# braun-steven/DAFNe

Hardware: AMD Instinct MI355X
Metric: images/sec on 1024x1024 DOTA tiles, R101-FPN (higher is better)
Workload: dtype bf16; 1 GPU; DOTA-1.0 1024x1024 R101-FPN bf16, batch 8 per GPU (per-GPU shard of configs[2]; the model BASELINE.json's metric names), uint8 tiles resident in HBM -> detections; per_gpu_batch=8, global_batch=8, classes=15, parallelism=dp1 (independent images, RCCL gather of detections), mode=pipelined

## Files before the change

### dafne_amd/_lib.py

```python
import ctypes
import os

_HERE = os.path.dirname(os.path.abspath(__file__))
LIB_PATH = os.environ.get("DAFNE_AMD_LIB") or os.path.join(_HERE, "libdafne_amd.so")
_lib = None

c_void_p = ctypes.c_void_p
c_int = ctypes.c_int
c_i64 = ctypes.c_int64
c_size_t = ctypes.c_size_t
c_double = ctypes.c_double
c_float = ctypes.c_float
c_u32 = ctypes.c_uint32
c_i32 = ctypes.c_int32


class LevelDesc(ctypes.Structure):
    _fields_ = [("d_logits", c_void_p), ("d_delta", c_void_p), ("d_center", c_void_p),
                ("d_ctrness", c_void_p), ("logits_ps", c_i32), ("delta_ps", c_i32),
                ("center_ps", c_i32), ("ctrness_ps", c_i32), ("H", c_i32), ("W", c_i32), ("stride", c_i32),
                ("scale", c_float)]


class DecodeParams(ctypes.Structure):
# ... 73 lines not shown
    "dafne_abi_version": (c_int, []),
    "dafne_last_error": (ctypes.c_char_p, []),
    "dafne_poly_iou_pairs_hip": (c_int, [c_void_p, c_void_p, c_i64, c_void_p, c_void_p]),
    "dafne_poly_nms_workspace_bytes": (c_size_t, [c_int, c_int]),
    "dafne_poly_nms_stats_offset": (c_size_t, [c_int, c_int, c_int]),
    "dafne_poly_nms_hip": (c_int, [c_void_p, c_int, c_double, c_void_p, c_void_p, c_void_p, c_size_t, c_int, c_void_p]),
    "dafne_poly_nms_batched_hip": (c_int, [c_void_p, c_void_p, c_int, c_int, c_double, c_int, c_void_p,
                                           c_void_p, c_void_p, c_size_t, c_int, c_void_p]),
    "dafne_poly_nms_f64_workspace_bytes": (c_size_t, [c_int, c_int]),
    "dafne_poly_nms_f64_batched_hip": (c_int, [c_void_p, c_void_p, c_int, c_int, c_double, c_int, c_void_p,
                                               c_void_p, c_void_p, c_size_t, c_int, c_void_p]),
    "dafne_hbb_nms_f64_workspace_bytes": (c_size_t, [c_int, c_int]),
    "dafne_hbb_nms_f64_batched_hip": (c_int, [c_void_p, c_void_p, c_int, c_int, c_double, c_void_p, c_void_p, c_void_p, c_size_t,
                                              c_void_p]),
    "dafne_select_over_all_levels_hip": (c_int, [c_void_p, c_void_p, c_void_p, c_void_p, c_int, c_int,
                                                 c_double, c_int, c_void_p, c_void_p, c_void_p, c_size_t,
                                                 c_int, c_void_p]),
    "dafne_decode_workspace_bytes": (c_size_t, [ctypes.POINTER(DecodeParams), ctypes.POINTER(LevelDesc)]),
    "dafne_decode_levels_hip": (c_int, [ctypes.POINTER(DecodeParams), ctypes.POINTER(LevelDesc)] +
                                [c_void_p] * 8 + [c_void_p, c_size_t, c_void_p]),
    "dafne_sort_quadrilateral_hip": (c_int, [c_void_p, c_void_p, c_i64, c_void_p]),
    "dafne_corner_chain_hip": (c_int, [ctypes.POINTER(ChainSeg), c_int, c_int, c_int, c_void_p, c_void_p]),
    "dafne_gather_detections_hip": (c_int, [c_void_p] * 10 + [c_int, c_int, c_int, c_int, c_void_p, c_void_p,
                                                             c_void_p]),
    "dafne_conv2d_nhwc_bf16_hip": (c_int, [ctypes.POINTER(ConvParams), ctypes.POINTER(ConvSeg), c_void_p]),
    "dafne_conv2d_nhwc_fp8w_hip": (c_int, [ctypes.POINTER(ConvParams), ctypes.POINTER(ConvSeg), c_void_p, c_float, c_void_p]),
    "dafne_conv2d_num_tiles": (c_int, [ctypes.POINTER(ConvParams), ctypes.POINTER(ConvSeg)]),
    "dafne_conv2d_fp8w_num_tiles": (c_int, [ctypes.POINTER(ConvParams), ctypes.POINTER(ConvSeg)]),
    "dafne_conv2d_fp8w_tiles_per_image": (c_int, [ctypes.POINTER(ConvParams), ctypes.POINTER(ConvSeg), c_void_p]),
    "dafne_resize_workspace_bytes": (c_size_t, [c_int, c_int, c_int]),
    "dafne_resize_bilinear_u8_hip": (c_int, [c_void_p, c_int, c_int, c_int, c_int, c_int, c_int, c_int, c_int, c_void_p,
                                             c_void_p, c_size_t, c_void_p]),
    "dafne_conv2d_kernel_id": (c_int, [ctypes.POINTER(ConvParams), ctypes.POINTER(ConvSeg)]),
    "dafne_conv2d_tiles_per_image": (c_int, [ctypes.POINTER(ConvParams), ctypes.POINTER(ConvSeg), c_void_p]),
    "dafne_groupnorm_finalize_hip": (c_int, [ctypes.POINTER(GnSeg), c_int, c_int, c_int, c_void_p, c_void_p,
                                             ctypes.c_float, c_void_p]),
    "dafne_conv2d_cout_pad": (c_int, [c_int]),
    "dafne_conv2d_tile_pixels": (c_int, [ctypes.POINTER(ConvParams), ctypes.POINTER(ConvSeg)]),
    "dafne_preprocess_image_hip": (c_int, [c_void_p, c_int, c_int, c_int, c_int, c_void_p,
                                           ctypes.POINTER(c_float), ctypes.POINTER(c_float), c_int, c_int,
                                           c_void_p, c_void_p]),
    "dafne_conv3x3_c64_hip": (c_int, [c_void_p, c_void_p, c_void_p, c_int, c_int, c_int, c_int, c_void_p, c_void_p]),
    "dafne_conv3x3_c256_ok": (c_int, [ctypes.POINTER(ConvParams), ctypes.POINTER(ConvSeg)]),
    "dafne_conv3x3_c256_num_tiles": (c_int, [ctypes.POINTER(ConvParams), ctypes.POINTER(ConvSeg)]),
    "dafne_conv3x3_c256_tiles_per_image": (c_int, [ctypes.POINTER(ConvParams), ctypes.POINTER(ConvSeg), c_void_p]),
    "dafne_conv3x3_c256_pair_hip": (c_int, [ctypes.POINTER(ConvParams), ctypes.POINTER(ConvSeg), c_void_p,
                                            ctypes.POINTER(ConvParams), ctypes.POINTER(ConvSeg), c_void_p, c_void_p, c_size_t, c_void_p]),
    "dafne_conv3x3_c256_scratch_bytes": (c_size_t, []),
    "dafne_conv3x3_c256_hip": (c_int, [ctypes.POINTER(ConvParams), ctypes.POINTER(ConvSeg), c_void_p, c_void_p, c_size_t, c_void_p]),
    "dafne_conv2d_wr_ok": (c_int, [ctypes.POINTER(ConvParams), ctypes.POINTER(ConvSeg)]),
    "dafne_conv2d_wr_splits": (c_int, [ctypes.POINTER(ConvParams), ctypes.POINTER(ConvSeg)]),
    "dafne_conv2d_wr_workspace_bytes": (c_size_t, [ctypes.POINTER(ConvParams), ctypes.POINTER(ConvSeg)]),
    "dafne_conv2d_wr_hip": (c_int, [ctypes.POINTER(ConvParams), ctypes.POINTER(ConvSeg), c_void_p, c_void_p, c_size_t, c_void_p]),
    "dafne_bottleneck_body_scratch_bytes": (c_size_t, []),
    "dafne_bottleneck_body_hip": (c_int, [c_void_p, c_void_p, c_void_p, c_void_p, c_void_p, c_void_p, c_int, c_int, c_int,
                                          c_void_p, c_void_p, c_void_p, c_size_t, c_void_p]),
    "dafne_bottleneck_body16_hip": (c_int, [c_void_p, c_void_p, c_void_p, c_void_p, c_void_p, c_void_p, c_int, c_int, c_int,
                                            c_void_p, c_void_p, c_void_p, c_size_t, c_void_p]),
    "dafne_bottleneck_tail_head_hip": (c_int, [c_void_p, c_void_p, c_void_p, c_void_p, c_void_p, c_int, c_int, c_int,
                                               c_void_p, c_void_p, c_void_p]),
    "dafne_bottleneck_tail_head_narrow_hip": (c_int, [c_void_p, c_void_p, c_void_p, c_void_p, c_void_p, c_int, c_int, c_int,
                                                      c_void_p, c_void_p, c_void_p]),
    "dafne_bottleneck_tail_head_mid_hip": (c_int, [c_void_p, c_void_p, c_void_p, c_void_p, c_void_p, c_int, c_int, c_int,
                                                   c_void_p, c_void_p, c_void_p]),
    "dafne_bottleneck_proj_tail_head_narrow_hip": (c_int, [c_void_p, c_void_p, c_void_p, c_void_p, c_void_p, c_void_p, c_int,
                                                           c_int, c_int, c_void_p, c_void_p, c_void_p]),
    "dafne_bottleneck_block_narrow_scratch_bytes": (c_size_t, []),
    "dafne_bottleneck_block_narrow_hip": (c_int, [c_void_p] * 7 + [c_int, c_int, c_int, c_void_p, c_void_p, c_void_p, c_size_t, c_void_p]),
    "dafne_bottleneck_block_narrow_s2_scratch_bytes": (c_size_t, []),
    "dafne_bottleneck_block_narrow_s2_hip": (c_int, [c_void_p] * 5 + [c_int, c_int, c_int, c_void_p, c_void_p, c_size_t, c_void_p]),
    "dafne_bottleneck_block_mid_scratch_bytes": (c_size_t, []),
    "dafne_bottleneck_block_mid_hip": (c_int, [c_void_p] * 6 + [c_int, c_int, c_int, c_void_p, c_void_p, c_void_p, c_size_t, c_void_p]),
    "dafne_stem_pool_hip": (c_int, [c_void_p, c_void_p, c_void_p, c_int, c_int, c_int, c_void_p, c_void_p]),
    "dafne_stem_pool_conv1_hip": (c_int, [c_void_p, c_void_p, c_void_p, c_void_p, c_void_p, c_int, c_int, c_int, c_void_p, c_void_p,
                                          c_void_p]),
    "dafne_maxpool3x3s2_nhwc_bf16_hip": (c_int, [c_void_p, c_void_p, c_int, c_int, c_int, c_int, c_void_p]),
    "dafne_groupnorm_relu_nhwc_bf16_hip": (c_int, [ctypes.POINTER(GnSeg), c_int, c_int, c_int, c_void_p, c_void_p,
                                                   c_void_p, c_void_p, c_float, c_void_p]),
    "dafne_relu_copy_bf16_hip": (c_int, [c_void_p, c_void_p, c_i64, c_void_p]),
    "dafne_scene_tiles_workspace_bytes": (c_size_t, [c_int]),
    "dafne_scene_tiles_u8_hip": (c_int, [ctypes.POINTER(SceneTile), c_int, c_int, c_void_p, c_void_p, c_size_t, c_void_p]),
    "dafne_scene_merge_workspace_bytes": (c_size_t, [c_int, c_int]),
    "dafne_scene_merge_rows_hip": (c_int, [c_void_p, c_void_p, c_int, c_int, c_void_p, c_int, c_int, ctypes.c_uint64, c_int,
                                           c_int, c_void_p, c_void_p, c_void_p, c_void_p, c_size_t, c_void_p]),
    "dafne_scene_merge_hbb_rows_hip": (c_int, [c_void_p, c_void_p, c_int, c_int, c_void_p, c_int, c_int, ctypes.c_uint64, c_int,
                                               c_int, c_void_p, c_void_p, c_void_p, c_void_p, c_size_t, c_void_p]),
    "dafne_scene_views_workspace_bytes": (c_size_t, [ctypes.POINTER(ViewSrc), c_int, c_int, c_int]),
    "dafne_scene_views_u8_hip": (c_int, [ctypes.POINTER(ViewSrc), c_int, c_int, c_int, c_void_p, c_void_p, c_size_t, c_void_p]),
    "dafne_scene_scaled_tiles_workspace_bytes": (c_size_t, [ctypes.POINTER(ScaledTile), c_int]),
    "dafne_scene_scaled_tiles_u8_hip": (c_int, [ctypes.POINTER(ScaledTile), c_int, c_int, c_void_p, c_void_p, c_size_t, c_void_p]),
    "dafne_scene_merge_rows_scaled_hip": (c_int, [c_void_p, c_void_p, c_int, c_int, c_void_p, c_void_p, c_int, c_int,
                                                  ctypes.c_uint64, c_int, c_int, c_void_p, c_void_p, c_void_p, c_void_p, c_size_t,
                                                  c_void_p]),
    "dafne_scene_merge_hbb_rows_scaled_hip": (c_int, [c_void_p, c_void_p, c_int, c_int, c_void_p, c_void_p, c_int, c_int,
                                                      ctypes.c_uint64, c_int, c_int, c_void_p, c_void_p, c_void_p, c_void_p,
                                                      c_size_t, c_void_p]),
    "dafne_tta_candidates_workspace_bytes": (c_size_t, [c_int, c_int]),
    "dafne_tta_candidates_hip": (c_int, [ctypes.POINTER(TtaView), c_int, c_int, c_int, c_int] + [c_void_p] * 10 + [c_size_t, c_void_p]),
    "dafne_scene_match_hip": (c_int, [c_void_p, c_void_p, c_int, c_void_p, c_void_p, c_int, c_int, c_void_p, c_void_p, c_void_p]),
    "dafne_scene_match_hbb_hip": (c_int, [c_void_p, c_void_p, c_int, c_void_p, c_void_p, c_int, c_int, c_void_p, c_void_p, c_void_p]),
    "dafne_scene_mark_workspace_bytes": (c_size_t, [c_int]),
    "dafne_scene_mark_hip": (c_int, [c_void_p, c_void_p, c_void_p, c_void_p, c_int, c_void_p, c_int, c_void_p, c_int, c_double,
                                     c_void_p, c_void_p, c_void_p, c_size_t, c_void_p]),
    "dafne_assign_targets_hip": (c_int, [ctypes.POINTER(TargetParams)] + [c_void_p] * 5 + [c_int] + [c_void_p] * 6),
    "dafne_losses_workspace_bytes": (c_size_t, [ctypes.POINTER(LossParams), ctypes.POINTER(LevelDesc)]),
    "dafne_losses_hip": (c_int, [ctypes.POINTER(LossParams), ctypes.POINTER(LevelDesc)] + [c_void_p] * 7 + [c_size_t, c_void_p]),
# ... 46 lines not shown
```

### dafne_amd/csrc/abi.hip

```cpp
#include "common.h"

namespace dafne {
char* err_buf() {
    static thread_local char buf[512] = {0};
    return buf;
}
}

extern "C" {
int dafne_abi_version(void) { return 151; }
const char* dafne_last_error(void) { return dafne::err_buf(); }
}
```

### dafne_amd/engine.py

```python
import ctypes

import torch

from . import _lib
from .engine_options import EngineOptions

BF16 = torch.bfloat16
STAGE_BLOCKS = {50: (3, 4, 6, 3), 101: (3, 4, 23, 3)}

F_RELU, F_RES, F_UP, F_F32, F_GN, F_GNIN, F_GNFIN, F_EXCL = 1, 2, 4, 8, 16, 32, 64, 128
F_FRAG16 = 256
F_RELU_INPUT = 512
FPN_IN_FEATURES = ("res3", "res4", "res5")


class Act:

    __slots__ = ("t", "n", "h", "w", "c")

    def __init__(self, n, h, w, c, device):
        self.t = torch.zeros(n, h + 2, w + 2, c, dtype=BF16, device=device)
        self.n, self.h, self.w, self.c = n, h, w, c

    def nchw_float(self):
# ... 174 lines not shown
    return 8 * a + 4 * cb + i


def pack_bneck16(w2, w3, w1):
    assert tuple(w2.shape) == (256, 2304) and w2.dtype == BF16
    assert tuple(w3.shape) == (1024, 256) and tuple(w1.shape) == (256, 1024) and w3.dtype == BF16 and w1.dtype == BF16
    perm = _bneck_row_perm16(w2.device)
    a0 = w2.reshape(8, 32, 72, 4, 8)[:, perm].reshape(8, 2, 16, 72, 4, 8).permute(0, 3, 1, 4, 2, 5)
    a1 = w3.reshape(4, 8, 32, 8, 4, 8)[:, :, perm].reshape(4, 8, 2, 16, 8, 4, 8).permute(0, 1, 4, 2, 5, 3, 6)
    a2 = w1.reshape(8, 32, 4, 8, 4, 8)[:, perm].reshape(8, 2, 16, 4, 8, 4, 8).permute(3, 0, 4, 1, 5, 2, 6)
    pb = torch.stack([a1, a2], dim=1).contiguous().reshape(-1)
    return torch.cat([a0.contiguous().reshape(-1), pb]).contiguous()


def bneck_weights(P, key, w2, w3, w1):
    f16 = P["options"].rp_mfma16
    fkey, other = (key + "bneck16", key + "bneck") if f16 else (key + "bneck", key + "bneck16")
    assert other not in P, "one conv_bneck form per model: %s" % other
    if fkey not in P:
        P[fkey] = pack_bneck16(w2, w3, w1) if f16 else pack_bneck(w2, w3, w1)
    return P[fkey], f16


def pack_conv3x3_frag(w):
    cout = w.shape[0]
    assert w.dim() == 2 and w.shape[1] == 2304 and cout % 256 == 0 and w.dtype == BF16
    return w.reshape(cout // 256, 8, 32, 144, 2, 8).permute(0, 1, 3, 4, 2, 5).contiguous().reshape(-1)


def pack_conv3x3_frag16(w):
    cout = w.shape[0]
    assert w.dim() == 2 and w.shape[1] == 2304 and cout % 256 == 0 and w.dtype == BF16
    return w.reshape(cout // 256, 8, 2, 16, 72, 4, 8).permute(0, 1, 4, 2, 5, 3, 6).contiguous().reshape(-1)


def pack_rp(w, options=None):
    options = options or EngineOptions.from_env()
    return (pack_conv3x3_frag16(w), F_FRAG16) if options.rp_mfma16 else (pack_conv3x3_frag(w), 0)


def rp_weights(P, key, wgt):
    f16 = P["options"].rp_mfma16
    fkey, other = (key + ".frag16", key + ".frag") if f16 else (key + ".frag", key + ".frag16")
    assert other not in P, "one resident-patch form per model: %s" % other
    if fkey not in P:
        P[fkey] = pack_rp(wgt, P["options"])[0]
    return P[fkey], f16


def pack_conv_frag(w):
    cout, k = w.shape
    assert w.dim() == 2 and cout % 256 == 0 and k % 64 == 0 and w.dtype == BF16
    return w.reshape(cout // 256, 8, 32, k // 16, 2, 8).permute(0, 1, 3, 4, 2, 5).contiguous().reshape(-1)


FP8_KERNELS = ("patch",)


_RP_SCRATCH = {}


def rp_scratch(device):
    key = str(device)
    if key not in _RP_SCRATCH:
        _RP_SCRATCH[key] = torch.empty(_lib.load().dafne_conv3x3_c256_scratch_bytes(), dtype=torch.uint8, device=device)
    return _RP_SCRATCH[key]


def pack_b2b_narrow(w3, w1, wsc=None):
    assert tuple(w3.shape) == (256, 64) and tuple(w1.shape) == (64, 256) and w3.dtype == BF16 and w1.dtype == BF16
    parts = [w3.reshape(8, 32, 4, 2, 8).permute(0, 2, 3, 1, 4).reshape(-1),
             w1.reshape(2, 32, 16, 2, 8).permute(0, 2, 3, 1, 4).reshape(-1)]
    if wsc is not None:
        assert tuple(wsc.shape) == (256, 64) and wsc.dtype == BF16
        parts.append(wsc.reshape(8, 32, 4, 2, 8).permute(0, 2, 3, 1, 4).reshape(-1))
    return torch.cat(parts).contiguous()


def pack_blk_narrow(w2, w3, w1=None, wsc=None):
    assert tuple(w2.shape) == (64, 576) and tuple(w3.shape) == (256, 64) and w2.dtype == BF16 and w3.dtype == BF16
    a2 = w2.reshape(2, 32, 36, 2, 8).permute(0, 2, 3, 1, 4).reshape(-1)

    def quarters(w):
        return w.reshape(2, 4, 32, 4, 2, 8).permute(0, 1, 3, 4, 2, 5).reshape(-1)
    if w1 is not None:
        assert tuple(w1.shape) == (64, 256) and w1.dtype == BF16
        a1 = w1.reshape(2, 32, 16, 2, 8).permute(0, 2, 3, 1, 4).reshape(-1)
    else:
        a1 = torch.zeros(2 * 16 * 64 * 8, dtype=BF16, device=w2.device)
    if wsc is not None:
        assert tuple(wsc.shape) == (256, 64) and wsc.dtype == BF16
        asc = quarters(wsc)
    else:
        asc = torch.zeros(256 * 64, dtype=BF16, device=w2.device)
    return torch.cat([a2, quarters(w3), a1, asc]).contiguous()


def pack_blk_mid(w2, w3, w1=None):
    assert tuple(w2.shape) == (128, 1152) and tuple(w3.shape) == (512, 128) and w2.dtype == BF16 and w3.dtype == BF16
    a2 = w2.reshape(4, 32, 72, 2, 8).permute(0, 2, 3, 1, 4).reshape(-1)
    a3 = w3.reshape(2, 8, 32, 8, 2, 8).permute(0, 1, 3, 4, 2, 5).reshape(-1)
    if w1 is not None:
        assert tuple(w1.shape) == (128, 512) and w1.dtype == BF16
        a1 = w1.reshape(4, 32, 32, 2, 8).permute(0, 2, 3, 1, 4).reshape(-1)
    else:
        a1 = torch.zeros(128 * 512, dtype=BF16, device=w2.device)
# ... 118 lines not shown
        rc = _lib.load().dafne_conv3x3_c256_pair_hip(ctypes.byref(a.prm), a.segs, _lib.ptr(a.wfrag), ctypes.byref(b.prm), b.segs,
                                                     _lib.ptr(b.wfrag), _lib.ptr(scr), scr.numel(), stream)
        if rc:
            _lib.check(rc, "dafne_conv3x3_c256_pair_hip")


WR_NOMINAL_BATCH = 8


def wr_takes(k, stride, cin, cout, npx):
    if k == 3:
        return stride in (1, 2) and npx <= 10000 and cin in (256, 512) and cout == cin
    if stride == 1:
        return (cin == 512 and cout == 2048 and npx <= 10000) or (cout == 256 and cin >= 1024 and npx <= 40000)
    return cin == 512 and cout == 256 and npx <= 40000


class WrWorkspace:

    def __init__(self, device):
        self.device, self.bytes, self.t = device, 0, None

    def need(self, nbytes):
        assert self.t is None
        self.bytes = max(self.bytes, int(nbytes))

    def tensor(self):
        if self.t is None:
            self.t = torch.zeros(max(self.bytes, 1 << 16), dtype=torch.uint8, device=self.device)
        return self.t


class WrCall:

    def __init__(self, conv, wfrag, ws):
        self.conv, self.wfrag, self.ws = conv, wfrag, ws
        self.prm, self.segs = conv.prm, conv.segs
        self.flops, self.bytes = conv.flops, conv.bytes
        L = _lib.load()
        self.splits = L.dafne_conv2d_wr_splits(ctypes.byref(self.prm), self.segs)
        assert self.splits >= 1
        ws.need(L.dafne_conv2d_wr_workspace_bytes(ctypes.byref(self.prm), self.segs))

    def kernel_name(self):
        return "conv_wr"

    def __call__(self, stream):
        w = self.ws.tensor()
        rc = _lib.load().dafne_conv2d_wr_hip(ctypes.byref(self.prm), self.segs, _lib.ptr(self.wfrag), _lib.ptr(w), w.numel(), stream)
        if rc:
            _lib.check(rc, "dafne_conv2d_wr_hip")


class FnCall:
    def __init__(self, fn, args, keep, name, flops=0, nbytes=0):
        self.fn, self.args, self.keep, self.name = fn, args, keep, name
        self.flops, self.bytes = flops, nbytes

    def kernel_name(self):
        return self.name

    def __call__(self, stream):
        rc = self.fn(*self.args, stream)
        if rc:
            _lib.check(rc, self.name)


def conv_out_hw(h, w, k, stride, pad):
    return (h + 2 * pad - k) // stride + 1, (w + 2 * pad - k) // stride + 1


class DensePlan:

    def __init__(self, weights, n, h, w, depth, num_classes, device, with_head=True, head_outputs=None, calib=None,
                 shared_gpu=False):
        assert h % 32 == 0 and w % 32 == 0
        self.shared_gpu = bool(shared_gpu)
        self._build(weights, n, h, w, depth, num_classes, device, with_head, head_outputs, calib)

    def _build(self, weights, n, h, w, depth, num_classes, device, with_head, head_outputs, calib):
        self.calib = calib
        self.n, self.h, self.w = n, h, w
        self.device = device
        self.calls = []
        self.flops = 0
        self.graph = None
        L = _lib.load()
        P = weights
        pool = Pool(device)
        self.pool = pool

        opt = P["options"]
        shared = self.shared_gpu and not opt.shared_excl
        act_q8 = P.get("act_q8") or {}
        wr_on = opt.conv_wr
        self.wr_ws = WrWorkspace(device)
        use_c64 = opt.conv_c64
        inplace_res = opt.inplace_res

        def res_dead(sc_, x_, b_):
            if not inplace_res or sc_ is None:
                return False
            if b_ == 0:
                return sc_ is not x_
            return not any(sc_ is f for f in feats.values())

        def conv(key, tin, k, stride, pad, flags, res=None, out=None, cout=None):
            wgt, bias = P[key]
            cin = tin.c
            cout = cout or wgt.shape[0]
            ho, wo = conv_out_hw(tin.h, tin.w, k, stride, pad)
            o = out or pool.get(n, ho, wo, cout)
            if (use_c64 and k == 3 and stride == 1 and pad == 1 and cin == 64 and cout == 64 and res is None
                    and (flags & ~F_RELU) == 0 and tuple(wgt.shape) == (64, 576) and bias is not None):
                fl = 2 * n * ho * wo * 64 * 576
                self.calls.append(FnCall(L.dafne_conv3x3_c64_hip,
                                         (_lib.ptr(tin.t), _lib.ptr(wgt), _lib.ptr(bias), n, ho, wo, 1 if flags & F_RELU else 0, _lib.ptr(o.t)),
                                         (tin, wgt, bias, o), "conv3x3_c64", flops=fl,
                                         nbytes=2 * n * ho * wo * 64 * 2 + wgt.numel() * 2))
                self.flops += fl
                return o
            q8 = P.get(key + ".fp8")
            fp8 = None
            if q8 is not None and k == 3 and stride == 1 and res is None and not (flags & (F_F32 | F_UP | F_RES)):
                if calib is not None:
                    self.calls.append(AmaxProbe(calib, key, [tin]))
                elif key in act_q8:
                    fp8 = (q8[1] / act_q8[key], act_q8[key])
            c = ConvCall(q8[0] if fp8 else wgt, bias, cin, cout, k, stride, pad, flags,
                         [(tin.t, o.t, res.t if res is not None else None, tin.h, tin.w, ho, wo)], n, fp8=fp8,
                         shared_gpu=shared)
            if (fp8 is None and wr_on and wr_takes(k, stride, cin, cout, WR_NOMINAL_BATCH * ho * wo) and bias is not None
                    and L.dafne_conv2d_wr_ok(ctypes.byref(c.prm), c.segs)):
                if key + ".wr" not in P:
                    P[key + ".wr"] = pack_conv_frag(wgt)
                w = WrCall(c, P[key + ".wr"], self.wr_ws)
                self.calls.append(w)
                self.flops += w.flops
                return o
            assert not (flags & F_RELU_INPUT), "only conv_wr rectifies its input on load (the caller checks wr_takes)"
            if fp8 is None and k == 3 and cin == 256 and opt.conv_rp and c.kernel_id() == 6 and c.rp_ok():
                wfrag, f16 = rp_weights(P, key, wgt)
                c = ConvCall(wgt, bias, cin, cout, k, stride, pad, flags,
                             [(tin.t, o.t, None, tin.h, tin.w, ho, wo)], n, wfrag=wfrag, shared_gpu=shared, frag16=f16)
            self.calls.append(c)
            self.flops += c.flops
            return o

        self.stem_in = torch.zeros(n, h + 6, w + 6, 4, dtype=BF16, device=device)
        wgt, bias = P["stem"]
        x = pool.get(n, h // 4, w // 4, 64)
        stem_flops = 2 * n * (h // 2) * (w // 2) * 64 * 7 * 7 * 3
        stem_y1 = None
        if opt.fuse_stem:
            c1 = P.get("res2.0.conv1")
            if (opt.fuse_stem_conv1 and c1 is not None and tuple(c1[0].shape) == (64, 64)
                    and c1[1] is not None):
                stem_y1 = pool.get(n, h // 4, w // 4, 64)
                c1_flops = 2 * n * (h // 4) * (w // 4) * 64 * 64
                fc = FnCall(L.dafne_stem_pool_conv1_hip, (_lib.ptr(self.stem_in), _lib.ptr(wgt), _lib.ptr(bias), _lib.ptr(c1[0]),
                                                          _lib.ptr(c1[1]), n, h, w, _lib.ptr(x.t), _lib.ptr(stem_y1.t)),
                            (self.stem_in, wgt, bias, c1[0], c1[1], x, stem_y1), "stem_pool_conv1", flops=stem_flops + c1_flops,
                            nbytes=n * ((h + 6) * (w + 6) * 8 + (h // 4) * (w // 4) * 256))
                self.calls.append(fc)
                self.flops += stem_flops + c1_flops
            else:
                fc = FnCall(L.dafne_stem_pool_hip, (_lib.ptr(self.stem_in), _lib.ptr(wgt), _lib.ptr(bias), n, h, w, _lib.ptr(x.t)),
                            (self.stem_in, wgt, bias, x), "stem_pool", flops=stem_flops,
                            nbytes=n * ((h + 6) * (w + 6) * 8 + (h // 4) * (w // 4) * 128))
                self.calls.append(fc)
                self.flops += stem_flops
        else:
            stem_out = pool.get(n, h // 2, w // 2, 64)
            c = ConvCall(wgt, bias, 4, 64, 7, 2, 3, F_RELU,
                         [(self.stem_in, stem_out.t, None, h + 6, w + 6, h // 2, w // 2)], n, shared_gpu=shared)
            self.calls.append(c)
            self.flops += c.flops
            self.calls.append(FnCall(L.dafne_maxpool3x3s2_nhwc_bf16_hip,
                                     (_lib.ptr(stem_out.t), _lib.ptr(x.t), n, h // 2, w // 2, 64),
                                     (stem_out, x), "maxpool"))
            pool.put(stem_out)

        feats = {}
        fuse_b2b, fuse_narrow, fuse_mid, fuse_bneck = opt.fuse_b2b, opt.b2b_narrow_on, opt.b2b_mid_on, opt.bneck_on
# ... 555 lines not shown
```

### include/dafne_amd.h

```cpp
#ifndef DAFNE_AMD_H
#define DAFNE_AMD_H

#include <stddef.h>
#include <stdint.h>

#ifdef __cplusplus
extern "C" {
#endif

#define DAFNE_OK 0
#define DAFNE_E_INVALID 1
#define DAFNE_E_WORKSPACE 2
#define DAFNE_E_HIP 3
#define DAFNE_E_UNSUPPORTED 4

int dafne_abi_version(void);
const char* dafne_last_error(void);

int dafne_poly_iou_pairs_hip(const double* d_p, const double* d_q, int64_t n,
                             double* d_out, void* stream);

size_t dafne_poly_nms_f64_workspace_bytes(int n_images, int m_cap);
int dafne_poly_nms_f64_batched_hip(const double* d_dets9, const int32_t* d_counts, int n_images, int m_cap,
                                   double thresh, int strict_hbb, int64_t* d_keep, int32_t* d_num_keep,
// ... 53 lines not shown
                                const int64_t* d_keep, const int32_t* d_num_keep,
                                const float* d_sizes, int do_postprocess, int n_images, int m_cap,
                                int k_cap, float* d_out, int32_t* d_out_counts, void* stream);

#define DAFNE_CONV_RELU 1u
#define DAFNE_CONV_RESIDUAL 2u
#define DAFNE_CONV_UPSAMPLE_ADD 4u
#define DAFNE_CONV_OUT_F32 8u
#define DAFNE_CONV_GN_STATS 16u
#define DAFNE_CONV_GN_INPUT 32u
#define DAFNE_CONV_GN_FINALIZE 64u
#define DAFNE_CONV_EXCLUSIVE 128u

#define DAFNE_CONV_FRAG16 256u
#define DAFNE_CONV_RELU_INPUT 512u

typedef struct dafne_conv_seg {
    const void* d_in;
    void* d_out;
    const void* d_res;
    int32_t Hin, Win, Hout, Wout;
} dafne_conv_seg;

typedef struct dafne_conv_params {
    int32_t n_images, n_segs;
    int32_t Cin, Cout, KH, KW, stride, pad;
    uint32_t flags;
    const void* d_weight;
    const float* d_bias;
    float* d_gn_partial;
    const float* d_in_gn_stats;
    const float* d_in_gn_gamma;
    const float* d_in_gn_beta;
    float* d_gn_stats_out;
    int32_t* d_gn_counters;
    float gn_eps;
} dafne_conv_params;

int dafne_conv2d_nhwc_bf16_hip(const dafne_conv_params* prm, const dafne_conv_seg* segs, void* stream);
int dafne_conv3x3_c256_ok(const dafne_conv_params* prm, const dafne_conv_seg* segs);
int dafne_conv3x3_c256_num_tiles(const dafne_conv_params* prm, const dafne_conv_seg* segs);
int dafne_conv3x3_c256_tiles_per_image(const dafne_conv_params* prm, const dafne_conv_seg* segs, int32_t* out);
int dafne_conv3x3_c256_pair_hip(const dafne_conv_params* prm_a, const dafne_conv_seg* segs_a, const void* d_wfrag_a,
                                const dafne_conv_params* prm_b, const dafne_conv_seg* segs_b, const void* d_wfrag_b,
                                void* d_scratch, size_t scratch_bytes, void* stream);
size_t dafne_conv3x3_c256_scratch_bytes(void);
int dafne_conv3x3_c256_hip(const dafne_conv_params* prm, const dafne_conv_seg* segs, const void* d_wfrag, void* d_scratch,
                           size_t scratch_bytes, void* stream);
int dafne_conv2d_wr_ok(const dafne_conv_params* prm, const dafne_conv_seg* segs);
int dafne_conv2d_wr_splits(const dafne_conv_params* prm, const dafne_conv_seg* segs);
size_t dafne_conv2d_wr_workspace_bytes(const dafne_conv_params* prm, const dafne_conv_seg* segs);
int dafne_conv2d_wr_hip(const dafne_conv_params* prm, const dafne_conv_seg* segs, const void* d_wfrag, void* d_workspace,
                        size_t workspace_bytes, void* stream);
int dafne_conv2d_nhwc_fp8w_hip(const dafne_conv_params* prm, const dafne_conv_seg* segs, const float* d_oscale,
                               float in_qscale, void* stream);
int dafne_conv2d_fp8w_num_tiles(const dafne_conv_params* prm, const dafne_conv_seg* segs);
int dafne_conv2d_fp8w_tiles_per_image(const dafne_conv_params* prm, const dafne_conv_seg* segs, int32_t* out);
int dafne_conv2d_cout_pad(int Cout);
int dafne_conv2d_tile_pixels(const dafne_conv_params* prm, const dafne_conv_seg* segs);
int dafne_conv2d_num_tiles(const dafne_conv_params* prm, const dafne_conv_seg* segs);
int dafne_conv2d_kernel_id(const dafne_conv_params* prm, const dafne_conv_seg* segs);
int dafne_conv2d_tiles_per_image(const dafne_conv_params* prm, const dafne_conv_seg* segs, int32_t* out);

int dafne_preprocess_image_hip(const uint8_t* d_img, int layout_hwc, int n_images, int H, int W,
                               const int32_t* d_valid_hw, const float* mean3, const float* std3,
                               int Hn, int Wn, void* d_out, void* stream);
size_t dafne_resize_workspace_bytes(int C, int H, int new_w);
int dafne_resize_bilinear_u8_hip(const uint8_t* d_in, int layout_hwc, int C, int H, int W, int new_h, int new_w,
                                 int hflip, int vflip, uint8_t* d_out, void* d_ws, size_t ws_bytes, void* stream);
int dafne_conv3x3_c64_hip(const void* d_in, const void* d_weight, const float* d_bias, int n_images, int H, int W, int relu,
                          void* d_out, void* stream);
int dafne_bottleneck_tail_head_hip(const void* d_in, const void* d_res, const void* d_wfrag, const float* d_bias3,
                                   const float* d_bias1, int n_images, int H, int W, void* d_out, void* d_next,
                                   void* stream);
size_t dafne_bottleneck_body_scratch_bytes(void);
int dafne_bottleneck_body_hip(const void* d_in, const void* d_res, const void* d_wfrag, const float* d_bias2,
                              const float* d_bias3, const float* d_bias1, int n_images, int H, int W, void* d_out,
                              void* d_next, void* d_scratch, size_t scratch_bytes, void* stream);
int dafne_bottleneck_body16_hip(const void* d_in, const void* d_res, const void* d_wfrag, const float* d_bias2,
                                const float* d_bias3, const float* d_bias1, int n_images, int H, int W, void* d_out,
                                void* d_next, void* d_scratch, size_t scratch_bytes, void* stream);
int dafne_bottleneck_tail_head_narrow_hip(const void* d_in, const void* d_res, const void* d_wfrag, const float* d_bias3,
                                          const float* d_bias1, int n_images, int H, int W, void* d_out, void* d_next,
                                          void* stream);
int dafne_bottleneck_tail_head_mid_hip(const void* d_in, const void* d_res, const void* d_wfrag, const float* d_bias3,
                                       const float* d_bias1, int n_images, int H, int W, void* d_out, void* d_next,
                                       void* stream);
int dafne_bottleneck_proj_tail_head_narrow_hip(const void* d_in, const void* d_x0, const void* d_wfrag, const float* d_bias3,
                                               const float* d_bias_sc, const float* d_bias1, int n_images, int H, int W,
                                               void* d_out, void* d_next, void* stream);
size_t dafne_bottleneck_block_narrow_scratch_bytes(void);
int dafne_bottleneck_block_narrow_hip(const void* d_in, const void* d_res, const void* d_wfrag, const float* d_bias2,
                                      const float* d_bias3, const float* d_bias_sc, const float* d_bias1, int n_images, int H, int W,
                                      void* d_out, void* d_next, void* d_scratch, size_t scratch_bytes, void* stream);
size_t dafne_bottleneck_block_narrow_s2_scratch_bytes(void);
int dafne_bottleneck_block_narrow_s2_hip(const void* d_in, const void* d_res, const void* d_wfrag, const float* d_bias2,
                                         const float* d_bias3, int n_images, int H, int W, void* d_out, void* d_scratch,
                                         size_t scratch_bytes, void* stream);
size_t dafne_bottleneck_block_mid_scratch_bytes(void);
int dafne_bottleneck_block_mid_hip(const void* d_in, const void* d_res, const void* d_wfrag, const float* d_bias2,
                                   const float* d_bias3, const float* d_bias1, int n_images, int H, int W, void* d_out,
                                   void* d_next, void* d_scratch, size_t scratch_bytes, void* stream);
int dafne_stem_pool_hip(const void* d_in, const void* d_weight, const float* d_bias, int n_images, int H, int W,
                        void* d_out, void* stream);
int dafne_stem_pool_conv1_hip(const void* d_in, const void* d_weight, const float* d_bias, const void* d_w1, const float* d_b1,
                              int n_images, int H, int W, void* d_out, void* d_out1, void* stream);
// ... 144 lines not shown
```

Baseline: 1420 images/sec.

## Add dedicated persistent MFMA GEMM kernel for 1x1 convs with 512->256 channels

Adds a new HIP kernel that runs 1x1 convolutions as a persistent GEMM. It keeps weights in registers, streams input pixels into LDS through a three-stage global_load_lds pipeline, uses XCD-aware tile walkers, and fuses bias, residual or top-down add, and ReLU into an LDS-staged epilogue. The engine routes only the stride-1 512->256 1x1 layer (the FPN res3 lateral) to this kernel, ahead of the existing conv_wr path. The aim is to cut the generic conv overhead for this layer, at the cost of a large amount of new inline-asm code that must hold correct wait counts and swizzles.

After: 1425 images/sec (median of 6 runs). No clear change (+0.4%).

```diff
diff --git a/dafne_amd/_lib.py b/dafne_amd/_lib.py
--- a/dafne_amd/_lib.py
+++ b/dafne_amd/_lib.py
@@ -149,6 +149,9 @@
     "dafne_conv2d_wr_splits": (c_int, [ctypes.POINTER(ConvParams), ctypes.POINTER(ConvSeg)]),
     "dafne_conv2d_wr_workspace_bytes": (c_size_t, [ctypes.POINTER(ConvParams), ctypes.POINTER(ConvSeg)]),
     "dafne_conv2d_wr_hip": (c_int, [ctypes.POINTER(ConvParams), ctypes.POINTER(ConvSeg), c_void_p, c_void_p, c_size_t, c_void_p]),
+    "dafne_conv1x1_gemm_ok": (c_int, [ctypes.POINTER(ConvParams), ctypes.POINTER(ConvSeg)]),
+    "dafne_conv1x1_gemm_tiles": (ctypes.c_longlong, [ctypes.POINTER(ConvParams), ctypes.POINTER(ConvSeg)]),
+    "dafne_conv1x1_gemm_hip": (c_int, [ctypes.POINTER(ConvParams), ctypes.POINTER(ConvSeg), c_void_p, c_void_p]),
     "dafne_bottleneck_body_scratch_bytes": (c_size_t, []),
     "dafne_bottleneck_body_hip": (c_int, [c_void_p, c_void_p, c_void_p, c_void_p, c_void_p, c_void_p, c_int, c_int, c_int,
                                           c_void_p, c_void_p, c_void_p, c_size_t, c_void_p]),
diff --git a/dafne_amd/csrc/abi.hip b/dafne_amd/csrc/abi.hip
--- a/dafne_amd/csrc/abi.hip
+++ b/dafne_amd/csrc/abi.hip
@@ -8,6 +8,6 @@
 }
 
 extern "C" {
-int dafne_abi_version(void) { return 151; }
+int dafne_abi_version(void) { return 152; }
 const char* dafne_last_error(void) { return dafne::err_buf(); }
 }
diff --git a/dafne_amd/csrc/conv1x1_gemm.hip b/dafne_amd/csrc/conv1x1_gemm.hip
--- /dev/null
+++ b/dafne_amd/csrc/conv1x1_gemm.hip
@@ -0,0 +1,444 @@
+#include <type_traits>
+
+#include "common.h"
+
+namespace {
+
+typedef __attribute__((ext_vector_type(8))) __bf16 bf16x8;
+typedef __attribute__((ext_vector_type(16))) float f32x16;
+typedef __attribute__((ext_vector_type(4))) float f32x4;
+typedef __attribute__((ext_vector_type(4))) unsigned u32x4;
+typedef __attribute__((ext_vector_type(2))) unsigned u32x2;
+typedef __attribute__((address_space(1))) void gvoid;
+typedef __attribute__((address_space(3))) void lvoid;
+
+template <int NW, int KR>
+struct Cfg {
+    static constexpr int NT = 64 * NW, CT = 32 * NW;
+    static constexpr int PX = KR ? 64 : 128;
+    static constexpr int PF = PX / 32;
+    static constexpr int KS = 32 / PF;
+    static constexpr int RB = KS * 32;
+    static constexpr int LPR = RB / 16;
+    static constexpr int RPP = 64 / LPR;
+    static constexpr int NP = 32 / NW;
+    static constexpr int STAGE = PX * RB;
+    static constexpr int NS = 3;
+    static constexpr int SLAB = PX * 128;
+    static constexpr int OFF_E = NS * STAGE;
+    static constexpr int SMEM = OFF_E + (NW / 2) * SLAB;
+    static constexpr int RN = PX / 16;
+    static_assert(STAGE == 32768 && SMEM <= 160 * 1024, "LDS");
+};
+
+struct GDev {
+    const char* in;
+    const char* wf;
+    const float* bias;
+    const char* res;
+    char* out;
+    int N, Hin, Win, Hout, Wout, Cin, Cout, stride;
+    int nk16;
+    int ptiles, ctiles;
+    int G;
+    int total_px;
+    unsigned flags;
+};
+
+__device__ __forceinline__ unsigned pack_bf16(float a, float b) {
+    typedef __attribute__((ext_vector_type(2))) float f32x2;
+    typedef __attribute__((ext_vector_type(2))) __bf16 bf16x2;
+    f32x2 v = {a, b};
+    bf16x2 r = __builtin_convertvector(v, bf16x2);
+    return __builtin_bit_cast(unsigned, r);
+}
+
+template <int I, int N, class F>
+__device__ __forceinline__ void static_for(F&& f) {
+    if constexpr (I < N) {
+        f(std::integral_constant<int, I>{});
+        static_for<I + 1, N>(f);
+    }
+}
+
+__device__ __forceinline__ void wait_vm(int n) {
+#define DAFNE_VM(k) case k: asm volatile("s_waitcnt vmcnt(" #k ")" ::: "memory"); break;
+    switch (n < 0 ? 0 : n) {
+        DAFNE_VM(0) DAFNE_VM(1) DAFNE_VM(2) DAFNE_VM(3) DAFNE_VM(4) DAFNE_VM(5) DAFNE_VM(6) DAFNE_VM(7)
+        DAFNE_VM(8) DAFNE_VM(9) DAFNE_VM(10) DAFNE_VM(11) DAFNE_VM(12) DAFNE_VM(13) DAFNE_VM(14) DAFNE_VM(15)
+        DAFNE_VM(16) DAFNE_VM(17) DAFNE_VM(18) DAFNE_VM(19) DAFNE_VM(20) DAFNE_VM(21) DAFNE_VM(22) DAFNE_VM(23)
+        DAFNE_VM(24) DAFNE_VM(25) DAFNE_VM(26) DAFNE_VM(27) DAFNE_VM(28) DAFNE_VM(29) DAFNE_VM(30) DAFNE_VM(31)
+        DAFNE_VM(32) DAFNE_VM(33) DAFNE_VM(34) DAFNE_VM(35) DAFNE_VM(36) DAFNE_VM(37) DAFNE_VM(38) DAFNE_VM(39)
+        DAFNE_VM(40) DAFNE_VM(41) DAFNE_VM(42) DAFNE_VM(43) DAFNE_VM(44) DAFNE_VM(45) DAFNE_VM(46) DAFNE_VM(47)
+        DAFNE_VM(48) DAFNE_VM(49) DAFNE_VM(50) DAFNE_VM(51) DAFNE_VM(52) DAFNE_VM(53) DAFNE_VM(54) DAFNE_VM(55)
+        DAFNE_VM(56) DAFNE_VM(57) DAFNE_VM(58) DAFNE_VM(59) DAFNE_VM(60) DAFNE_VM(61) DAFNE_VM(62)
+        default: asm volatile("s_waitcnt vmcnt(63)" ::: "memory"); break;
+    }
+#undef DAFNE_VM
+}
+
+template <int NW, int KR>
+__global__ void __launch_bounds__(64 * NW, NW == 8 ? 2 : 1) conv1x1_gemm_kernel(GDev P) {
+    using C = Cfg<NW, KR>;
+    constexpr int PF = C::PF, KS = C::KS;
+    constexpr int NA = KR ? KR : 16;
+    extern __shared__ __attribute__((aligned(16))) char lds[];
+    const int tid = threadIdx.x;
+    const int lane = tid & 63;
+    const int wave = __builtin_amdgcn_readfirstlane(tid >> 6);
+    const int frow = lane & 31, half = lane >> 5;
+    const unsigned lds_base = (unsigned)(size_t)(__attribute__((address_space(3))) char*)lds;
+
+    const int xcd = blockIdx.x & 7, bidx = blockIdx.x >> 3;
+    const int ct = bidx % P.ctiles;
+    const int walker = (bidx / P.ctiles) * 8 + xcd;
+    if (walker >= P.ptiles) return;
+    const int ntl = (P.ptiles - walker + P.G - 1) / P.G;
+    const int SPT = KR ? KR / 16 : (P.nk16 + 7) >> 3;
+    const int T = ntl * SPT;
+
+    const int HW = P.Hout * P.Wout;
+    auto coords = [&](int gp, int& img, int& oy, int& ox) __attribute__((always_inline)) {
+        gp = gp < P.total_px ? gp : P.total_px - 1;
+        img = gp / HW;
+        const int m = gp - img * HW;
+        oy = m / P.Wout;
+        ox = m - oy * P.Wout;
+    };
+
+    int issued = 0;
+    int mP0 = 0, mP1 = 0, mW = 0, mR = 0;
+
+    unsigned pofs[C::NP];
+    auto set_pofs = [&](int pt) __attribute__((always_inline)) {
+#pragma unroll
+        for (int ii = 0; ii < C::NP; ii++) {
+            const int r = (wave * C::NP + ii) * C::RPP + lane / C::LPR;
+            int img, oy, ox;
+            coords(pt * C::PX + r, img, oy, ox);
+            const unsigned g = (unsigned)((img * (P.Hin + 2) + oy * P.stride + 1) * (P.Win + 2) + ox * P.stride + 1);
+            const int p = lane % C::LPR;
+            pofs[ii] = g * (unsigned)(P.Cin * 2) + (unsigned)(((p & 16) | ((p & 15) ^ (r & 15))) * 16);
+        }
+    };
+    int ig = 0, ij = 0, itile = 0, islot = 0;
+    auto issue_P = [&]() __attribute__((always_inline)) {
+        if (ig < T) {
+            const unsigned so = (unsigned)ij * (unsigned)C::RB;
+#pragma unroll
+            for (int ii = 0; ii < C::NP; ii++)
+                __builtin_amdgcn_global_load_lds((gvoid*)(P.in + (size_t)(pofs[ii] + so)),
+                                                 (lvoid*)(lds + islot * C::STAGE + (wave * C::NP + ii) * 1024), 16, 0, 0);
+            issued += C::NP;
+            ig++;
+            if (++ij == SPT) {
+                ij = 0;
+                itile++;
+                if (ig < T) set_pofs(walker + itile * P.G);
+            }
+        }
+        islot = islot == C::NS - 1 ? 0 : islot + 1;
+    };
+
+    const char* wbase = P.wf + ((size_t)(ct * NW + wave) * P.nk16) * 1024;
+    const unsigned voff = (unsigned)(lane * 16);
+    bf16x8 wa[NA];
+#pragma unroll
+    for (int k = 0; k < NA; k++) wa[k] = bf16x8{};
+    auto load_A = [&](int k16, bf16x8& dst) __attribute__((always_inline)) {
+        const char* sb = wbase + (size_t)(k16 < P.nk16 ? k16 : P.nk16 - 1) * 1024;
+        asm volatile("global_load_dwordx4 %0, %1, %2" : "+v"(dst) : "v"(voff), "s"(sb) : "memory");
+    };
+    auto issue_W = [&](int j, auto PARN) __attribute__((always_inline)) {
+        constexpr int pn = decltype(PARN)::value;
+        static_for<0, 8>([&](auto I) __attribute__((always_inline)) { load_A(8 * j + decltype(I)::value, wa[(pn * 8 + decltype(I)::value) % NA]); });
+        issued += 8;
+        mW = issued;
+    };
+
+    unsigned bs[8];
+#pragma unroll
+    for (int s = 0; s < 8; s++) bs[s] = (unsigned)(frow * C::RB + (((2 * s + half) ^ (frow & 15)) * 16));
+    bf16x8 bfr[2][PF];
+    auto bread = [&](unsigned stage_addr, auto SS, bf16x8 (&b)[PF]) {
+        constexpr int s = decltype(SS)::value;
+        const unsigned ad = stage_addr + bs[s & 7];
+        if constexpr (PF == 4) {
+            asm volatile("ds_read_b128 %0, %4\n\tds_read_b128 %1, %4 offset:8192\n\tds_read_b128 %2, %4 offset:16384\n\tds_read_b128 %3, %4 offset:24576"
+                         : "=&v"(b[0]), "=&v"(b[1]), "=&v"(b[2]), "=&v"(b[3])
+                         : "v"(ad)
+                         : "memory");
+        } else if constexpr (s < 8) {
+            asm volatile("ds_read_b128 %0, %2\n\tds_read_b128 %1, %2 offset:16384" : "=&v"(b[0]), "=&v"(b[1]) : "v"(ad) : "memory");
+        } else {
+            asm volatile("ds_read_b128 %0, %2 offset:256\n\tds_read_b128 %1, %2 offset:16640" : "=&v"(b[0]), "=&v"(b[1]) : "v"(ad) : "memory");
+        }
+    };
+    auto tie_b = [&](bf16x8 (&b)[PF]) {
+#pragma unroll
+        for (int k = 0; k < PF; k++) asm volatile("" : "+v"(b[k]));
+    };
+    auto barrier = [&]() __attribute__((always_inline)) {
+        __builtin_amdgcn_sched_barrier(0);
+        asm volatile("s_waitcnt lgkmcnt(0)" ::: "memory");
+        __builtin_amdgcn_s_barrier();
+        __builtin_amdgcn_sched_barrier(0);
+    };
+
+    f32x16 acc[PF];
+#pragma unroll
+    for (int b = 0; b < PF; b++)
+#pragma unroll
+        for (int k = 0; k < 16; k++) acc[b][k] = 0.f;
+
+    const bool relu = P.flags & DAFNE_CONV_RELU;
+    const float relu_lo = relu ? 0.f : -__builtin_inff();
+    const bool has_res = P.flags & DAFNE_CONV_RESIDUAL, has_up = P.flags & DAFNE_CONV_UPSAMPLE_ADD;
+    const bool has_add = has_res || has_up;
+
+    auto issue_R = [&](int pt) __attribute__((always_inline)) {
+        constexpr int RUNS = C::RN / (NW / 2);
+#pragma unroll
+        for (int a = 0; a < RUNS; a++) {
+            const int pp = wave * RUNS + a;
+            const int px = pp * 8 + (lane >> 3);
+            int img, oy, ox;
+            coords(pt * C::PX + px, img, oy, ox);
+            const size_t rpix = has_up ? ((size_t)(img * (P.Hout / 2 + 2) + oy / 2 + 1) * (P.Wout / 2 + 2) + ox / 2 + 1)
+                                       : ((size_t)(img * (P.Hout + 2) + oy + 1) * (P.Wout + 2) + ox + 1);
+            const char* src = P.res + (rpix * P.Cout + ct * C::CT) * 2 + ((lane & 7) ^ ((px >> 1) & 7)) * 16;
+#pragma unroll
+            for (int sl = 0; sl < NW / 2; sl++)
+                __builtin_amdgcn_global_load_lds((gvoid*)(src + sl * 128), (lvoid*)(lds + C::OFF_E + sl * C::SLAB + pp * 1024), 16, 0, 0);
+        }
+        issued += C::RN;
+        mR = issued;
+    };
+
+    f32x4 bia[4];
+#pragma unroll
+    for (int g = 0; g < 4; g++) {
+        bia[g] = f32x4{};
+        const float* bp = P.bias + ct * C::CT + wave * 32 + 8 * g + 4 * half;
+        asm volatile("global_load_dwordx4 %0, %1, off" : "+v"(bia[g]) : "v"(bp) : "memory");
+    }
+    issued += 4;
+    if constexpr (KR > 0) {
+        static_for<0, KR>([&](auto K) __attribute__((always_inline)) { load_A(decltype(K)::value, wa[decltype(K)::value]); });
+        issued += KR;
+    }
+    const int mBA = issued;
+    if constexpr (KR == 0) issue_W(0, std::integral_constant<int, 0>{});
+    set_pofs(walker);
+    issue_P();
+    mP0 = issued;
+    issue_P();
+    mP1 = issued;
+    wait_vm(issued - mBA);
+#pragma unroll
+    for (int g = 0; g < 4; g++) asm volatile("" : "+v"(bia[g]));
+    if constexpr (KR > 0) {
+#pragma unroll
+        for (int k = 0; k < KR; k++) asm volatile("" : "+v"(wa[k]));
+    }
+
+    auto epilogue = [&](int pt) __attribute__((always_inline)) {
+        if (has_add) {
+            wait_vm(issued - mR);
+            barrier();
+        }
+        const unsigned ebase = lds_base + C::OFF_E + (wave >> 1) * C::SLAB + frow * 128 + 8 * half;
+#pragma unroll
+        for (int g = 0; g < 4; g++) {
+            const unsigned ea = ebase + ((((wave & 1) * 4 + g) ^ ((frow >> 1) & 7)) * 16);
+            u32x2 r[PF];
+#pragma unroll
+            for (int b = 0; b < PF; b++) r[b] = u32x2{0u, 0u};
+            if (has_add) {
+#pragma unroll
+                for (int b = 0; b < PF; b++) asm volatile("ds_read_b64 %0, %1" : "+v"(r[b]) : "v"(ea + b * 4096) : "memory");
+                asm volatile("s_waitcnt lgkmcnt(0)" ::: "memory");
+#pragma unroll
+                for (int b = 0; b < PF; b++) asm volatile("" : "+v"(r[b]));
+            }
+#pragma unroll
+            for (int b = 0; b < PF; b++) {
+                const float v0 = fmaxf((acc[b][4 * g] + bia[g][0]) + __uint_as_float(r[b].x << 16), relu_lo);
+                const float v1 = fmaxf((acc[b][4 * g + 1] + bia[g][1]) + __uint_as_float(r[b].x & 0xffff0000u), relu_lo);
+                const float v2 = fmaxf((acc[b][4 * g + 2] + bia[g][2]) + __uint_as_float(r[b].y << 16), relu_lo);
+                const float v3 = fmaxf((acc[b][4 * g + 3] + bia[g][3]) + __uint_as_float(r[b].y & 0xffff0000u), relu_lo);
+                u32x2 o;
+                o.x = pack_bf16(v0, v1);
+                o.y = pack_bf16(v2, v3);
+                asm volatile("ds_write_b64 %0, %1" :: "v"(ea + b * 4096), "v"(o) : "memory");
+            }
+        }
+        barrier();
+#pragma unroll
+        for (int h = 0; h < C::PX / (8 * NW); h++) {
+            const int px = h * 8 * NW + (tid >> 3);
+            const int q = tid & 7;
+            int img, oy, ox;
+            coords(pt * C::PX + px, img, oy, ox);
+            char* dst = P.out + (((size_t)(img * (P.Hout + 2) + oy + 1) * (P.Wout + 2) + ox + 1) * P.Cout + ct * C::CT) * 2 + q * 16;
+            const unsigned la = lds_base + C::OFF_E + px * 128 + ((q ^ ((px >> 1) & 7)) * 16);
+            u32x4 v[NW / 2];
+#pragma unroll
+            for (int sl = 0; sl < NW / 2; sl++) {
+                v[sl] = u32x4{};
+                asm volatile("ds_read_b128 %0, %1" : "+v"(v[sl]) : "v"(la + sl * C::SLAB) : "memory");
+            }
+            asm volatile("s_waitcnt lgkmcnt(0)" ::: "memory");
+#pragma unroll
+            for (int sl = 0; sl < NW / 2; sl++) {
+                asm volatile("" : "+v"(v[sl]));
+                asm volatile("global_store_dwordx4 %0, %1, off\n\ts_nop 1" :: "v"(dst + sl * 128), "v"(v[sl]) : "memory");
+            }
+        }
+        issued += C::RN;
+    };
+
+    int j = 0, cpt = walker, cslot = 0;
+    auto consume = [&](int g, auto PAR) __attribute__((always_inline)) {
+        constexpr int par = decltype(PAR)::value;
+        constexpr int AB = KR == 0 ? par * 8 : (KR == 32 ? par * 16 : 0);
+        wait_vm(issued - (KR == 0 && mW > mP0 ? mW : mP0));
+        if constexpr (KR == 0) {
+#pragma unroll
+            for (int k = 0; k < 8; k++) asm volatile("" : "+v"(wa[AB + k]));
+        }
+        barrier();
+        if constexpr (KR == 0) {
+            if (g + 1 < T) issue_W(j + 1 == SPT ? 0 : j + 1, std::integral_constant<int, par ^ 1>{});
+        }
+        issue_P();
+        mP0 = mP1;
+        mP1 = issued;
+        if (j == 0 && has_add) issue_R(cpt);
+        const bool full = KR > 0 || P.nk16 - 8 * j >= 8;
+        const unsigned sa = lds_base + (unsigned)(cslot * C::STAGE);
+        bread(sa, std::integral_constant<int, 0>{}, bfr[0]);
+        static_for<0, KS>([&](auto SS) __attribute__((always_inline)) {
+            constexpr int s = decltype(SS)::value;
+            if constexpr (s + 1 < KS) {
+                bread(sa, std::integral_constant<int, s + 1>{}, bfr[(s + 1) & 1]);
+                if constexpr (PF == 4) asm volatile("s_waitcnt lgkmcnt(4)" ::: "memory");
+                else asm volatile("s_waitcnt lgkmcnt(2)" ::: "memory");
+            } else {
+                asm volatile("s_waitcnt lgkmcnt(0)" ::: "memory");
+            }
+            tie_b(bfr[s & 1]);
+            __builtin_amdgcn_sched_barrier(0);
+            if (s < 4 || full) {
+#pragma unroll
+                for (int b = 0; b < PF; b++) acc[b] = __builtin_amdgcn_mfma_f32_32x32x16_bf16(wa[AB + s], bfr[s & 1][b], acc[b], 0, 0, 0);
+            }
+            __builtin_amdgcn_sched_barrier(0);
+        });
+        cslot = cslot == C::NS - 1 ? 0 : cslot + 1;
+        if (j == SPT - 1) {
+            epilogue(cpt);
+#pragma unroll
+            for (int b = 0; b < PF; b++)
+#pragma unroll
+                for (int k = 0; k < 16; k++) acc[b][k] = 0.f;
+            j = 0;
+            cpt += P.G;
+        } else {
+            j++;
+        }
+    };
+    for (int g = 0; g < T; g += 2) {
+        consume(g, std::integral_constant<int, 0>{});
+        if (g + 1 < T) consume(g + 1, std::integral_constant<int, 1>{});
+    }
+}
+
+int g_build(GDev& D, const dafne_conv_params* prm, const dafne_conv_seg* segs, int* nw, int* kr, int* grid, const char** why) {
+    *why = nullptr;
+    if (!prm || !segs) { *why = "null argument"; return 0; }
+    const unsigned allowed = DAFNE_CONV_RELU | DAFNE_CONV_RESIDUAL | DAFNE_CONV_UPSAMPLE_ADD | DAFNE_CONV_EXCLUSIVE;
+    if (prm->n_segs != 1) { *why = "one segment"; return 0; }
+    if (prm->flags & ~allowed) { *why = "flags"; return 0; }
+    if ((prm->flags & DAFNE_CONV_RESIDUAL) && (prm->flags & DAFNE_CONV_UPSAMPLE_ADD)) { *why = "residual and top-down add"; return 0; }
+    if (prm->KH != 1 || prm->KW != 1 || prm->pad != 0) { *why = "1x1, pad 0"; return 0; }
+    if (prm->stride != 1 && prm->stride != 2) { *why = "stride"; return 0; }
+    if (prm->Cin < 64 || prm->Cin % 64 || prm->Cout < 128 || prm->Cout % 128) { *why = "Cin % 64, Cout % 128"; return 0; }
+    if (!prm->d_bias) { *why = "bias"; return 0; }
+    const dafne_conv_seg& S = segs[0];
+    if (prm->n_images < 1 || S.Hout < 1 || S.Wout < 1 || (long long)S.Hout * S.Wout > (1 << 20)) { *why = "size"; return 0; }
+    if (S.Hout != (S.Hin - 1) / prm->stride + 1 || S.Wout != (S.Win - 1) / prm->stride + 1) { *why = "geometry"; return 0; }
+    if ((prm->flags & DAFNE_CONV_UPSAMPLE_ADD) && ((S.Hout & 1) || (S.Wout & 1))) { *why = "top-down add on an odd map"; return 0; }
+    const long long in_bytes = (long long)prm->n_images * (S.Hin + 2) * (S.Win + 2) * prm->Cin * 2;
+    const long long total = (long long)prm->n_images * S.Hout * S.Wout;
+    if (in_bytes > 0xffffffffll || total > (1ll << 21)) { *why = "too large"; return 0; }
+    D.in = (const char*)S.d_in; D.out = (char*)S.d_out; D.res = (const char*)S.d_res;
+    D.bias = (const float*)prm->d_bias;
+    D.N = prm->n_images; D.Hin = S.Hin; D.Win = S.Win; D.Hout = S.Hout; D.Wout = S.Wout;
+    D.Cin = prm->Cin; D.Cout = prm->Cout; D.stride = prm->stride;
+    D.nk16 = D.Cin / 16;
+    D.total_px = (int)total;
+    D.flags = prm->flags;
+    *nw = D.Cout % 256 == 0 ? 8 : 4;
+    *kr = D.Cin == 512 ? 32 : D.Cin == 256 ? 16 : 0;
+    const int px = *kr ? 64 : 128;
+    D.ptiles = (int)((total + px - 1) / px);
+    D.ctiles = D.Cout / (32 * *nw);
+    int cus = 0;
+    if (dafne::device_cus(&cus)) cus = 256;
+    int m = cus / (8 * D.ctiles);
+    if (m > (D.ptiles + 7) / 8) m = (D.ptiles + 7) / 8;
+    if (m < 1) m = 1;
+    D.G = 8 * m;
+    *grid = 8 * D.ctiles * m;
+    return 1;
+}
+
+template <int NW, int KR>
+int g_launch(const GDev& D, int grid, hipStream_t stream) {
+    using C = Cfg<NW, KR>;
+    DAFNE_MAX_LDS_ONCE(C::SMEM, (const void*)conv1x1_gemm_kernel<NW, KR>);
+    hipLaunchKernelGGL((conv1x1_gemm_kernel<NW, KR>), dim3((unsigned)grid), dim3(C::NT), C::SMEM, stream, D);
+    return dafne::check_launch("conv1x1_gemm");
+}
+
+}
+
+extern "C" {
+
+int dafne_conv1x1_gemm_ok(const dafne_conv_params* prm, const dafne_conv_seg* segs) {
+    GDev D;
+    int nw, kr, grid;
+    const char* why;
+    return g_build(D, prm, segs, &nw, &kr, &grid, &why);
+}
+
+long long dafne_conv1x1_gemm_tiles(const dafne_conv_params* prm, const dafne_conv_seg* segs) {
+    GDev D;
+    int nw, kr, grid;
+    const char* why;
+    if (!g_build(D, prm, segs, &nw, &kr, &grid, &why)) return 0;
+    return ((long long)D.ptiles * D.ctiles << 32) | (long long)grid;
+}
+
+int dafne_conv1x1_gemm_hip(const dafne_conv_params* prm, const dafne_conv_seg* segs, const void* d_wfrag, void* stream) {
+    GDev D;
+    int nw, kr, grid;
+    const char* why;
+    if (!g_build(D, prm, segs, &nw, &kr, &grid, &why))
+        return dafne::fail(why && why[0] == 'n' ? DAFNE_E_INVALID : DAFNE_E_UNSUPPORTED, "conv1x1_gemm: %s", why ? why : "?");
+    if (!d_wfrag || !D.in || !D.out) return dafne::fail(DAFNE_E_INVALID, "conv1x1_gemm: null argument");
+    if ((D.flags & (DAFNE_CONV_RESIDUAL | DAFNE_CONV_UPSAMPLE_ADD)) && !D.res) return dafne::fail(DAFNE_E_INVALID, "conv1x1_gemm: residual flag without d_res");
+    D.wf = (const char*)d_wfrag;
+    hipStream_t s = (hipStream_t)stream;
+    if (nw == 8) {
+        if (kr == 32) return g_launch<8, 32>(D, grid, s);
+        if (kr == 16) return g_launch<8, 16>(D, grid, s);
+        return g_launch<8, 0>(D, grid, s);
+    }
+    if (kr == 32) return g_launch<4, 32>(D, grid, s);
+    if (kr == 16) return g_launch<4, 16>(D, grid, s);
+    return g_launch<4, 0>(D, grid, s);
+}
+
+}
diff --git a/dafne_amd/engine.py b/dafne_amd/engine.py
--- a/dafne_amd/engine.py
+++ b/dafne_amd/engine.py
@@ -250,6 +250,12 @@
     cout, k = w.shape
     assert w.dim() == 2 and cout % 256 == 0 and k % 64 == 0 and w.dtype == BF16
     return w.reshape(cout // 256, 8, 32, k // 16, 2, 8).permute(0, 1, 3, 4, 2, 5).contiguous().reshape(-1)
+
+
+def pack_gemm1x1_frag(w):
+    cout, k = w.shape
+    assert w.dim() == 2 and cout % 128 == 0 and k % 64 == 0 and w.dtype == BF16
+    return w.reshape(cout // 32, 32, k // 16, 2, 8).permute(0, 2, 3, 1, 4).contiguous().reshape(-1)
 
 
 FP8_KERNELS = ("patch",)
@@ -474,6 +480,36 @@
             _lib.check(rc, "dafne_conv2d_wr_hip")
 
 
+def gemm1x1_takes(stride, cin, cout, npx):
+    return (stride, cin, cout) in GEMM1X1_LAYERS and npx <= GEMM1X1_MAX_NPX
+
+
+GEMM1X1_LAYERS = frozenset([
+    (1, 512, 256),
+])
+GEMM1X1_MAX_NPX = WR_NOMINAL_BATCH * 128 * 128
+
+
+class Gemm1x1Call:
+
+    def __init__(self, conv, wfrag):
+        self.conv, self.wfrag = conv, wfrag
+        self.prm, self.segs = conv.prm, conv.segs
+        self.flops, self.bytes = conv.flops, conv.bytes
+
+    def kernel_name(self):
+        return "conv1x1_gemm"
+
+    def tiles(self):
+        v = _lib.load().dafne_conv1x1_gemm_tiles(ctypes.byref(self.prm), self.segs)
+        return v >> 32, v & 0xffffffff
+
+    def __call__(self, stream):
+        rc = _lib.load().dafne_conv1x1_gemm_hip(ctypes.byref(self.prm), self.segs, _lib.ptr(self.wfrag), stream)
+        if rc:
+            _lib.check(rc, "dafne_conv1x1_gemm_hip")
+
+
 class FnCall:
     def __init__(self, fn, args, keep, name, flops=0, nbytes=0):
         self.fn, self.args, self.keep, self.name = fn, args, keep, name
@@ -552,6 +588,15 @@
             c = ConvCall(q8[0] if fp8 else wgt, bias, cin, cout, k, stride, pad, flags,
                          [(tin.t, o.t, res.t if res is not None else None, tin.h, tin.w, ho, wo)], n, fp8=fp8,
                          shared_gpu=shared)
+            if (fp8 is None and wr_on and k == 1 and pad == 0 and bias is not None
+                    and gemm1x1_takes(stride, cin, cout, WR_NOMINAL_BATCH * ho * wo)
+                    and L.dafne_conv1x1_gemm_ok(ctypes.byref(c.prm), c.segs)):
+                if key + ".g1" not in P:
+                    P[key + ".g1"] = pack_gemm1x1_frag(wgt)
+                g1 = Gemm1x1Call(c, P[key + ".g1"])
+                self.calls.append(g1)
+                self.flops += g1.flops
+                return o
             if (fp8 is None and wr_on and wr_takes(k, stride, cin, cout, WR_NOMINAL_BATCH * ho * wo) and bias is not None
                     and L.dafne_conv2d_wr_ok(ctypes.byref(c.prm), c.segs)):
                 if key + ".wr" not in P:
diff --git a/include/dafne_amd.h b/include/dafne_amd.h
--- a/include/dafne_amd.h
+++ b/include/dafne_amd.h
@@ -129,6 +129,9 @@
 size_t dafne_conv2d_wr_workspace_bytes(const dafne_conv_params* prm, const dafne_conv_seg* segs);
 int dafne_conv2d_wr_hip(const dafne_conv_params* prm, const dafne_conv_seg* segs, const void* d_wfrag, void* d_workspace,
                         size_t workspace_bytes, void* stream);
+int dafne_conv1x1_gemm_ok(const dafne_conv_params* prm, const dafne_conv_seg* segs);
+long long dafne_conv1x1_gemm_tiles(const dafne_conv_params* prm, const dafne_conv_seg* segs);
+int dafne_conv1x1_gemm_hip(const dafne_conv_params* prm, const dafne_conv_seg* segs, const void* d_wfrag, void* stream);
 int dafne_conv2d_nhwc_fp8w_hip(const dafne_conv_params* prm, const dafne_conv_seg* segs, const float* d_oscale,
                                float in_qscale, void* stream);
 int dafne_conv2d_fp8w_num_tiles(const dafne_conv_params* prm, const dafne_conv_seg* segs);
```
